# cesar-rocha/niwqg

Measured on NVIDIA B200. Metric: fp64 grid-point-steps/sec (coupled NIW-QG), higher is better.
Workload: dtype f64

## Files before the change

### niwqg_b200/csrc/common.cuh

```cuda
#pragma once
#include <cuda_runtime.h>
#include "fft_core.cuh"

#define NIWQG_PW_THREADS 256
#define NIWQG_PW_BLOCKS (148 * 4)

__host__ __device__ __forceinline__ int sidx(int i, int N) { return i < (N >> 1) ? i : i - N; }

struct Grid {
    int N;
    double dk;
    int ncl;
    int h;
    int rank;
    int sym;
};
__host__ __device__ __forceinline__ int grid_kx(const Grid& g, int lc) {
    if (!g.sym) return lc;
    if (lc < g.h) return g.rank * g.h + lc;
    if (g.rank == 0 && lc == g.h) return g.N >> 1;
    return g.N - (g.rank * g.h + lc - g.h);
}
__host__ __device__ __forceinline__ int grid_partner(const Grid& g, int lc) {
    if (!g.sym) return (g.N - lc) & (g.N - 1);
    if (g.rank == 0 && (lc == 0 || lc == g.h)) return lc;
    return lc < g.h ? lc + g.h : lc - g.h;
}
__host__ __device__ __forceinline__ void grid_owner(int N, int h, int kx, int& rank, int& lc) {
    const int H = N >> 1;
    if (kx < H) { rank = kx / h; lc = kx % h; }
    else if (kx == H) { rank = 0; lc = h; }
    else { const int m = N - kx; rank = m / h; lc = h + m % h; }
}

template <int K>
__device__ __forceinline__ void block_reduce_store(double (&s)[K], double* __restrict__ partials) {
    __shared__ double sh[NIWQG_PW_THREADS / 32][K];
    const int lane = threadIdx.x & 31, warp = threadIdx.x >> 5;
#pragma unroll
    for (int k = 0; k < K; ++k) {
        double x = s[k];
#pragma unroll
        for (int off = 16; off > 0; off >>= 1) x += __shfl_down_sync(0xffffffffu, x, off);
        if (lane == 0) sh[warp][k] = x;
    }
    __syncthreads();
    if (threadIdx.x < K) {
        double x = 0.0;
#pragma unroll
        for (int w = 0; w < NIWQG_PW_THREADS / 32; ++w) x += sh[w][threadIdx.x];
        partials[((size_t)blockIdx.y * gridDim.x + blockIdx.x) * K + threadIdx.x] = x;
    }
}

template <int K>
__device__ __forceinline__ void block_reduce_max_store(double (&s)[K], double* __restrict__ partials) {
    __shared__ double shm[NIWQG_PW_THREADS / 32][K];
    const int lane = threadIdx.x & 31, warp = threadIdx.x >> 5;
#pragma unroll
    for (int k = 0; k < K; ++k) {
        double x = s[k];
#pragma unroll
        for (int off = 16; off > 0; off >>= 1) x = fmax(x, __shfl_down_sync(0xffffffffu, x, off));
        if (lane == 0) shm[warp][k] = x;
    }
    __syncthreads();
// ... 8 lines not shown
```

### niwqg_b200/csrc/fft2d.cuh

```cuda
#pragma once
#include <cooperative_groups.h>
#include <cuda.h>
#include "common.cuh"

namespace cg = cooperative_groups;

enum {
    PRO_NONE = 0,
    PRO_REAL_IN,
    PRO_IK,
    PRO_IL,
    PRO_NEG_WV2,
    PRO_WV4,
    PRO_UV,
    PRO_IK_CONJ,
    PRO_IL_CONJ,
};
enum { EPI_NONE = 0, EPI_REAL_OUT };

struct FftArgs {
    const void* in;
    void* out;
    const cd* tw;
    const cd* twc;
    int pro, epi;
    int conj_in, conj_out;
    double scale, scale_im;
    double dk;
    int pf_groups;
    Grid g;
    int nlines;
    int pitch;
    int xmap_in, xmap_out;
    int xchunk;
    int deint_in, deint_out;
    int push;
    int nyl_shift;
    int panel;
    cd* peer[8];
    size_t mstride;
    int tma_in;
    int one_cta_per_sm;
    int variant;
    const cd *in2, *in3;
    double ld_scale;
};
enum {
    LD_NONE = 0,
    LD_WAVEPV,
    LD_UQVQ,
};

__device__ __forceinline__ size_t panel_offset(const FftArgs& a, int yl, int lc) {
    int cs = 0;
    while ((1 << cs) < a.panel) ++cs;
    const int rp = ((yl & (a.panel - 1)) << (a.nyl_shift - cs)) | (yl >> cs);
    return ((((size_t)(lc >> 2)) << a.nyl_shift) + rp) * 4 + (lc & 3);
}

template <int N, bool COL, bool NAT>
__device__ __forceinline__ size_t fft_index(const FftArgs& a, int xmap, int line, int n) {
    if (NAT) return COL ? (size_t)n * N + line : (size_t)line * N + n;
    if (COL) return (size_t)n * a.pitch + line;
    if (!xmap) return (size_t)line * N + n;
    int r, lc;
    grid_owner(N, a.g.h, n, r, lc);
    if (a.panel) return (size_t)r * a.xchunk + panel_offset(a, line, lc);
    return (size_t)r * a.xchunk + (size_t)line * a.g.ncl + lc;
}
template <bool COL>
__device__ __forceinline__ void fft_kykx(const FftArgs& a, int line, int n, int& ky, int& kx) {
    if (COL) { ky = n; kx = a.g.sym ? grid_kx(a.g, line) : line; } else { ky = line; kx = n; }
}

template <int N, int PRO>
__device__ __forceinline__ cd fft_prologue_one(const FftArgs& a, int row, int col, cd x) {
    const double k = a.dk * (double)sidx(col, N), l = a.dk * (double)sidx(row, N);
    if (PRO == PRO_IK) return make_double2(-k * x.y, k * x.x);
    if (PRO == PRO_IL) return make_double2(-l * x.y, l * x.x);
    if (PRO == PRO_IL_CONJ) return make_double2(l * x.y, -l * x.x);
    if (PRO == PRO_IK_CONJ) return make_double2(k * x.y, -k * x.x);
    if (PRO == PRO_NEG_WV2) { const double w = -(k * k + l * l); return make_double2(w * x.x, w * x.y); }
    if (PRO == PRO_WV4) { double w = k * k + l * l; w = w * w; return make_double2(w * x.x, w * x.y); }
// ... 172 lines not shown
        const cd* __restrict__ p2 = a.in3 + i0;
#pragma unroll
        for (int b = 0; b < fftc::E; b += 4) {
            cd x0[4], x1[4], x2[4];
#pragma unroll
            for (int i = 0; i < 4; ++i) {
                x0[i] = __ldg(p0 + (b + i) * TL::TPF); x1[i] = __ldg(p1 + (b + i) * TL::TPF); x2[i] = __ldg(p2 + (b + i) * TL::TPF);
            }
#pragma unroll
            for (int i = 0; i < 4; ++i) {
                const double im = x1[i].x * x2[i].y - x1[i].y * x2[i].x;
                v[b + i] = make_double2(x0[i].x * x0[i].x + x0[i].y * x0[i].y, a.ld_scale * (-2.0 * im));
            }
        }
        for (int t = tid; t < TL::TWLEN; t += TL::T) smtw[t] = a.tw[t];
        tma_done = true;
    }
    if constexpr (LD == LD_UQVQ) {
        static_assert(!COL && NAT && C == 1, "loader passes are one-tile row passes");
        const size_t i0 = mbase + (size_t)group * W * N + (size_t)w * M + j;
        const cd* __restrict__ p0 = (const cd*)a.in + i0;
        const cd* __restrict__ p1 = a.in2 + i0;
#pragma unroll
        for (int b = 0; b < fftc::E; b += 8) {
            cd x0[8], x1[8];
#pragma unroll
            for (int i = 0; i < 8; ++i) { x0[i] = __ldg(p0 + (b + i) * TL::TPF); x1[i] = __ldg(p1 + (b + i) * TL::TPF); }
#pragma unroll
            for (int i = 0; i < 8; ++i) v[b + i] = make_double2(x0[i].x * x1[i].x, x0[i].y * x1[i].x);
        }
        for (int t = tid; t < TL::TWLEN; t += TL::T) smtw[t] = a.tw[t];
        tma_done = true;
    }
    if constexpr (LD == LD_NONE && COL && NAT && C == 1 && M >= 256) {
        if (a.tma_in & 1) {
            const unsigned bar = smem_u32(smtw + TL::TWLEN);
            if (tid == 0) {
                mbar_init(bar, 1);
                asm volatile("fence.proxy.async.shared::cta;" ::: "memory");
            }
            __syncthreads();
            if (tid == 0) {
                mbar_expect_tx(bar, (unsigned)(W * M * sizeof(cd)));
#pragma unroll
                for (int b4 = 0; b4 < M / 256; ++b4)
                    tma_load_2d(smem_u32(smem + (size_t)b4 * 256 * W), &tmap, group * W * 2, (int)blockIdx.y * N + b4 * 256, bar);
            }
            for (int t = tid; t < TL::TWLEN; t += TL::T) smtw[t] = a.tw[t];
            mbar_wait(bar, 0);
#pragma unroll
            for (int e = 0; e < fftc::E; ++e) v[e] = smem[(size_t)(j + e * TL::TPF) * W + w];
            __syncthreads();
            tma_done = true;
        }
    }
    if constexpr (LD == LD_NONE && !COL && NAT && C == 1 && M * W == 4096) {
        if ((a.tma_in & 2) && a.pro != PRO_REAL_IN) {
            const unsigned bar = smem_u32(smtw + TL::TWLEN);
            if (tid == 0) {
                mbar_init(bar, 1);
                asm volatile("fence.proxy.async.shared::cta;" ::: "memory");
            }
            __syncthreads();
            if (tid == 0) {
                mbar_expect_tx(bar, (unsigned)(W * M * sizeof(cd)));
                bulk_load(smem_u32(smem), (const cd*)a.in + mbase + (size_t)group * W * N, (unsigned)(W * M * sizeof(cd)), bar);
// ... 426 lines not shown
```

### niwqg_b200/csrc/fft_split.cuh

```cuda
#pragma once
#include "fft2d.cuh"

struct SplitPArgs {
    const cd* in;
    cd* out[3];
    int pro[3];
    int nout;
    int conj_in;
    double scale;
    double dk;
    const cd* twc;
};

template <int N, int PRO>
__device__ __forceinline__ cd split_prologue(double dk, int row, int col, cd x) {
    FftArgs a{};
    a.dk = dk;
    return fft_prologue_one<N, PRO>(a, row, col, x);
}

template <int N, bool DIT>
__global__ void __launch_bounds__(256, 2) k_split_p(SplitPArgs a) {
    constexpr int R = 16, M = N / R, Nh = N / 2;
    const int lane = threadIdx.x & 31, warp = threadIdx.x >> 5;
// ... 56 lines not shown
            fftc::apply_twiddles<R, 1>(u, wy);
        }
        cd* out = a.out[o];
#pragma unroll
        for (int q = 0; q < R; ++q) {
            cd x = u[q];
            if (DIT) { x.x *= a.scale; x.y *= a.scale; }
            out[(size_t)(DIT ? m + M * q : q * M + m) * N + col] = x;
        }
    }
}

template <int M, int W, int R, bool DIT>
__global__ void __launch_bounds__(W * M / 16, 2) k_fft_colsub2(FftArgs a) {
    using TL = Tile<M, W, R, true>;
    constexpr int N = TL::N;
    extern __shared__ __align__(128) unsigned char smem_raw[];
    cd* smem = reinterpret_cast<cd*>(smem_raw);
    cd* smtw = smem + (size_t)W * TL::LINE;
    const int tid = threadIdx.x, w = tid % W, j = tid / W;
    const int q = (int)(blockIdx.x % R), group = (int)(blockIdx.x / R);
    const int line = group * W + w;
    const cd* in = (const cd*)a.in;
    cd v[fftc::E];
#pragma unroll
    for (int e = 0; e < fftc::E; ++e) {
        const int jj = j + e * TL::TPF;
        v[e] = in[(size_t)(DIT ? R * jj + q : q * M + jj) * N + line];
    }
    for (int t = tid; t < TL::TWLEN; t += TL::T) smtw[t] = a.tw[t];
    fft_stages<M, W, R, true, true, true, 1>(v, j, w, q, smem, smtw, a, line, 0);
}

template <int N>
static cudaError_t split_set_attrs() {
    constexpr int M = N / 16, W = 4096 / M;
    using TL = Tile<M, W, 16, true>;
    static bool attr_set[64] = {};
    int dev = 0;
    cudaGetDevice(&dev);
    if (dev < 64 && !attr_set[dev]) {
        cudaError_t e = cudaFuncSetAttribute(k_fft_colsub2<M, W, 16, false>, cudaFuncAttributeMaxDynamicSharedMemorySize, (int)TL::SMEM);
        if (e != cudaSuccess) return e;
        e = cudaFuncSetAttribute(k_fft_colsub2<M, W, 16, true>, cudaFuncAttributeMaxDynamicSharedMemorySize, (int)TL::SMEM);
        if (e != cudaSuccess) return e;
        attr_set[dev] = true;
    }
    return cudaSuccess;
}

template <int N, bool DIT>
static cudaError_t launch_split_colsub(const FftArgs& a, cudaStream_t st) {
    constexpr int M = N / 16, W = 4096 / M;
    using TL = Tile<M, W, 16, true>;
    cudaError_t e = split_set_attrs<N>();
    if (e != cudaSuccess) return e;
    FftArgs b = a;
    b.deint_out = DIT ? 1 : 0;
    k_fft_colsub2<M, W, 16, DIT><<<dim3((N / W) * 16, 1), TL::T, TL::SMEM, st>>>(b);
    return cudaGetLastError();
}

template <int N, int LD>
static cudaError_t launch_split_rows_loader(const FftArgs& a, cudaStream_t st) {
    constexpr int Nh = N / 2, W = 4096 / Nh;
    using TL = Tile<Nh, W, 1, false>;
    static bool attr_set[64] = {};
    int dev = 0;
    cudaGetDevice(&dev);
    if (dev >= 64 || !attr_set[dev]) {
        cudaError_t e = cudaFuncSetAttribute(k_fft_pass<Nh, W, 1, false, true, LD>, cudaFuncAttributeMaxDynamicSharedMemorySize, (int)TL::SMEM);
        if (e != cudaSuccess) return e;
        if (dev < 64) attr_set[dev] = true;
    }
    CUtensorMap tmap;
    memset(&tmap, 0, sizeof tmap);
    FftArgs b = a;
    b.tma_in = 0; b.pf_groups = 0;
    k_fft_pass<Nh, W, 1, false, true, LD><<<dim3(a.nlines / W, 1, 1), TL::T, TL::SMEM, st>>>(b, tmap);
    return cudaGetLastError();
}

template <int N, bool DIT>
static cudaError_t launch_split_p(const SplitPArgs& a, cudaStream_t st) {
    k_split_p<N, DIT><<<dim3(N / 2 / 128, N / 16, 1), 256, 0, st>>>(a);
    return cudaGetLastError();
}
```

### niwqg_b200/csrc/kernels_family.cuh

```cuda
#pragma once
#include "common.cuh"

enum {
    MF_WAVE_PV   = 1 << 0,
    MF_QL_ADV    = 1 << 1,
    MF_YBJ       = 1 << 2,
    MF_FIX00     = 1 << 3,
    MF_HAS_LAP2  = 1 << 4,
    MF_NO_WRITE  = 1 << 5,
    MF_SKIP_P1   = 1 << 6,
    MF_SKIP_P2   = 1 << 7,
    MF_SPEC_BUDGET = 1 << 8,
    MF_P1_BY_LOADER = 1 << 9,
};


__device__ __forceinline__ cd cexp_d(cd z) {
    double s, c;
    sincos(z.y, &s, &c);
    const double e = exp(z.x);
    return make_double2(e * c, e * s);
}
__device__ __forceinline__ cd cdiv_d(cd a, cd b) {
    if (fabs(b.x) >= fabs(b.y)) {
        const double r = b.y / b.x, d = b.x + b.y * r;
        return make_double2((a.x + a.y * r) / d, (a.y - a.x * r) / d);
    } else {
        const double r = b.x / b.y, d = b.x * r + b.y;
        return make_double2((a.x * r + a.y) / d, (a.y * r - a.x) / d);
    }
}

__device__ void etdrk4_point(cd ch, double dt, cd& E, cd& E2, cd& Q, cd& f0, cd& fab, cd& fc) {
    E = cexp_d(ch);
    E2 = cexp_d(make_double2(0.5 * ch.x, 0.5 * ch.y));
    cd sQ = make_double2(0, 0), s0 = sQ, sab = sQ, sc = sQ;
    for (int jj = 1; jj <= 32; ++jj) {
        double sr, cr;
        sincospi(2.0 * (double)jj / 32.0, &sr, &cr);
        const cd LR = make_double2(ch.x + cr, ch.y + sr);
        const cd LR2 = cmul(LR, LR), LR3 = cmul(LR2, LR);
        const cd eh = cexp_d(make_double2(0.5 * LR.x, 0.5 * LR.y));
        const cd e1 = cexp_d(LR);
        sQ = cadd(sQ, cdiv_d(make_double2(eh.x - 1.0, eh.y), LR));
        cd t = cmul(e1, make_double2(4.0 - 3.0 * LR.x + LR2.x, -3.0 * LR.y + LR2.y));
        s0 = cadd(s0, cdiv_d(make_double2(-4.0 - LR.x + t.x, -LR.y + t.y), LR3));
// ... 139 lines not shown
        if (a.qwh) a.qwh[i1] = make_double2(qwb.x * fl1, qwb.y * fl1);
        if (!self) {
            a.ph[i2] = make_double2(ph1.x, -ph1.y);
            a.qs[i2] = make_double2(Hq.x + qw.y, -Hq.y + qw.x);
            if (a.qwh) a.qwh[i2] = make_double2(qwb.x * fl2, -qwb.y * fl2);
        }
    }
    if (a.partials) block_reduce_store<SI_COUNT>(s, a.partials);
}

__global__ void k_spec_uvq(Grid g, const cd* __restrict__ qh, cd* __restrict__ uvq) {
    const int N = g.N, H = N >> 1, NC = g.ncl;
    const size_t npts = (size_t)N * NC, mb = (size_t)blockIdx.y * npts;
    const size_t total = (size_t)(H + 1) * NC;
    for (size_t t = (size_t)blockIdx.x * blockDim.x + threadIdx.x; t < total; t += (size_t)gridDim.x * blockDim.x) {
        const int ky = (int)(t / NC), lc = (int)(t % NC);
        const int kyp = (N - ky) & (N - 1), lcp = grid_partner(g, lc);
        if (kyp == ky && lcp < lc) continue;
        const int kx = grid_kx(g, lc), kxp = grid_kx(g, lcp);
        const size_t i1 = mb + (size_t)ky * NC + lc, i2 = mb + (size_t)kyp * NC + lcp;
        const double k1 = g.dk * (double)sidx(kx, N), l1 = g.dk * (double)sidx(ky, N);
        const double k2 = g.dk * (double)sidx(kxp, N), l2 = g.dk * (double)sidx(kyp, N);
        const double wv2 = __dadd_rn(__dmul_rn(k1, k1), __dmul_rn(l1, l1));
        const double wv2i = (wv2 != 0.0) ? 1.0 / wv2 : 0.0;
        const cd q1 = qh[i1], q2 = qh[i2];
        const cd G1 = make_double2(-wv2i * q1.x, -wv2i * q1.y), G2 = make_double2(-wv2i * q2.x, -wv2i * q2.y);
        cd o1, o2;
        pack_uv_general(k1, l1, k2, l2, G1, G2, o1, o2);
        uvq[i1] = o1;
        if (i1 != i2) uvq[i2] = o2;
    }
}

enum {
    SD_G1 = 0,
    SD_G2,
    SD_X1,
    SD_X2,
    SD_PHI_R, SD_PHI_I,
    SD_QPC_R, SD_QPC_I,
    SD_PHI2,
    SD_GRAD2,
    SD_LAP2,
    SD_J_R, SD_J_I,
    SD_Q2,
    SD_QP2,
    SD_QP3,
    SD_COUNT
};

struct PhysArgs {
    size_t npts;
    int flags;
    double nu4w, nuw, muw;
    const cd *uv, *qs, *phi, *phix, *phiy, *lapphi, *lap2phi, *uvq;
    cd *P1, *P2;
    double* partials;
};

__global__ void __launch_bounds__(NIWQG_PW_THREADS) k_phys_rhs(PhysArgs a) {
    const size_t mb = (size_t)blockIdx.y * a.npts;
    double s[SD_COUNT];
#pragma unroll
    for (int k = 0; k < SD_COUNT; ++k) s[k] = 0.0;
    const bool ybj = (a.flags & MF_YBJ) != 0, wr = !(a.flags & MF_NO_WRITE);
    const bool nosums = ybj || (a.flags & MF_SKIP_P1);
    for (size_t i = (size_t)blockIdx.x * blockDim.x + threadIdx.x; i < a.npts; i += (size_t)gridDim.x * blockDim.x) {
        const cd uv = a.uv[mb + i], qs = a.qs[mb + i];
        const cd phi = a.phi[mb + i], px = a.phix[mb + i], py = a.phiy[mb + i];
        const double u = uv.x, v = uv.y, q = qs.x, qpsi = qs.x - qs.y;
        const cd J = make_double2(u * px.x + v * py.x, u * px.y + v * py.y);
        cd Jadv = J;
        if (a.flags & MF_QL_ADV) {
            const cd w = a.uvq[mb + i];
            Jadv = make_double2(w.x * px.x + w.y * py.x, w.x * px.y + w.y * py.y);
        }
        if (wr) {
            if (!ybj && !(a.flags & (MF_SKIP_P1 | MF_P1_BY_LOADER))) a.P1[mb + i] = make_double2(u * q, v * q);
            if (!(a.flags & MF_SKIP_P2))
                a.P2[mb + i] = make_double2(-Jadv.x + 0.5 * phi.y * qpsi, -Jadv.y - 0.5 * phi.x * qpsi);
        }
        if (nosums) continue;
        s[SD_PHI_R] += phi.x; s[SD_PHI_I] += phi.y;
        s[SD_QPC_R] += qpsi * phi.x; s[SD_QPC_I] += -qpsi * phi.y;
        s[SD_PHI2] += phi.x * phi.x + phi.y * phi.y;
        s[SD_GRAD2] += px.x * px.x + px.y * px.y + py.x * py.x + py.y * py.y;
        s[SD_J_R] += Jadv.x; s[SD_J_I] += Jadv.y;
        s[SD_Q2] += q * q;
        s[SD_QP2] += qpsi * qpsi;
        s[SD_QP3] += qpsi * qpsi * qpsi;
        if (a.flags & MF_SPEC_BUDGET) continue;
        const cd lp = a.lapphi[mb + i];
        cd diss = make_double2(a.nuw * lp.x - a.muw * phi.x, a.nuw * lp.y - a.muw * phi.y);
        if (a.flags & MF_HAS_LAP2) {
            const cd l2 = a.lap2phi[mb + i];
            diss.x += -a.nu4w * l2.x; diss.y += -a.nu4w * l2.y;
        }
        s[SD_G1] += qpsi * (phi.x * lp.y - phi.y * lp.x);
        s[SD_G2] += lp.x * J.x + lp.y * J.y;
        s[SD_X1] += -(diss.y * J.x - diss.x * J.y);
        s[SD_X2] += 0.5 * (diss.x * phi.x + diss.y * phi.y) * qpsi;
        s[SD_LAP2] += lp.x * lp.x + lp.y * lp.y;
    }
    if (!nosums) block_reduce_store<SD_COUNT>(s, a.partials);
}

__global__ void __launch_bounds__(256) k_finalize(const double* __restrict__ partials, int nblk, int K, double* __restrict__ out, int is_max) {
    __shared__ double sh[16][17];
    const int m = blockIdx.x, k = threadIdx.x & 15, part = threadIdx.x >> 4;
    const double* p = partials + (size_t)m * nblk * K;
    double x = is_max ? -1.0e300 : 0.0;
// ... 282 lines not shown
```

### niwqg_b200/csrc/niwqg_b200.cu

```cuda
#include <cstdio>
#include <cstdlib>
#include <cstring>
#include <cmath>
#include <string>
#include <vector>
#include <dlfcn.h>
#include <nccl.h>
#include "../../include/niwqg_b200.h"
#include "fft2d.cuh"
#include "fft_split.cuh"
#include "kernels_family.cuh"
#include "kernels_fused.cuh"
#include "kernels_qg.cuh"
#include "kernels_ic.cuh"

static std::string g_create_error;

#define CK(call)                                                                                   \
    do {                                                                                           \
        cudaError_t e__ = (call);                                                                  \
        if (e__ != cudaSuccess) {                                                                  \
            char buf__[512];                                                                       \
            snprintf(buf__, sizeof buf__, "%s:%d: %s: %s", __FILE__, __LINE__, #call, cudaGetErrorString(e__)); \
            h->err = buf__;                                                                        \
            return -2;                                                                             \
        }                                                                                          \
    } while (0)

struct niwqg_handle {
    niwqg_params p;
    int N = 0, B = 1, model = 0, flags = 0;
    bool qg = false;
// ... 17 lines not shown
    cd *ph = nullptr, *qwh = nullptr;
    cd *phi = nullptr, *phix = nullptr, *phiy = nullptr, *lapphi = nullptr, *lap2phi = nullptr;
    cd *uv = nullptr, *qs = nullptr, *uvq = nullptr;
    cd *W = nullptr, *P1 = nullptr, *P2 = nullptr;
    double* rscratch = nullptr;
    double *part = nullptr, *sumsD = nullptr, *sumsE = nullptr, *sumsX = nullptr, *sumsI = nullptr, *scal = nullptr,
           *stagev = nullptr;
    bool q_set = false, phi_set = false;
    int deintC = 1, deintM = 0;
    int rank = 0, nranks = 1, nyl = 0, ncl = 0;
    Grid g{};
    double Mg = 0;
    cd *X = nullptr, *Y = nullptr;
    static constexpr int NLANE = 2;
    cd* Yp[NLANE][2] = {};
    cd* peerY[NLANE][2][8] = {};
    bool p2p = false;
    int ybuf[NLANE] = {0, 0};
    double* bar[NLANE] = {nullptr, nullptr};
    cudaStream_t lane_stream[NLANE] = {nullptr, nullptr};
    ncclComm_t lane_comm[NLANE] = {nullptr, nullptr};
    cudaEvent_t ev_fork = nullptr, ev_join = nullptr;
    struct StepGraph { cudaGraphExec_t exec = nullptr; int cq = 0, cp = 0, cc = 0; long long launches = 0; };
    StepGraph graphs[8];
    bool use_graphs = false;
    int direct_steps = 0;
    int exchange = 0;
    cd* Xl[NLANE] = {nullptr, nullptr};
    ncclComm_t comm = nullptr;
    bool col3 = false;
    cd* S3[2] = {nullptr, nullptr};
    cd* tw_c3 = nullptr;
    int split = 0;
    cd* T[3] = {nullptr, nullptr, nullptr};
    cd *tw_half = nullptr, *tw_m = nullptr;
    cudaStream_t copy_stream = nullptr, copy_out = nullptr;
    cudaEvent_t ev_up_done = nullptr, ev_up_free = nullptr, ev_dn_ready = nullptr, ev_dn_done[2] = {nullptr, nullptr};
    bool up_free_rec = false, dn_done_rec[2] = {false, false};
    void* stage_in = nullptr;
    void* pre_buf[2] = {nullptr, nullptr};
    cudaEvent_t pre_done[2] = {nullptr, nullptr}, pre_free[2] = {nullptr, nullptr};
    bool pre_staged[2] = {false, false}, pre_free_rec[2] = {false, false};
    void* stage_out[2] = {nullptr, nullptr};
    double* pin = nullptr;
    int slab_panel = 0;
    int flag_barrier = 1;
    unsigned bar_epoch[NLANE] = {0, 0};
    bool prof = false;
    struct ProfRec { int kind; cudaEvent_t a, b; };
    std::vector<ProfRec> prof_recs;
    std::vector<cudaEvent_t> prof_pool;
    size_t prof_used = 0;
};

enum { PK_FFT_ROW = 0, PK_FFT_COL, PK_PHYS, PK_SPEC, PK_SMALL, PK_COMM, PK_FFT_P, PK_FFT_ROWLD, PK_FFT_ROWLD2, PK_COUNT };

static cudaEvent_t prof_event(niwqg_handle* h) {
    if (h->prof_used == h->prof_pool.size()) {
        cudaEvent_t e;
        cudaEventCreate(&e);
        h->prof_pool.push_back(e);
    }
    return h->prof_pool[h->prof_used++];
}
struct ProfScope {
    niwqg_handle* h; int kind; cudaEvent_t a;
// ... 101 lines not shown
    const int r = threadIdx.x;
    if (r >= nranks) return;
    unsigned v;
    do {
        asm volatile("ld.acquire.sys.global.u32 %0, [%1];" : "=r"(v) : "l"(flags + r) : "memory");
        if (v < epoch) __nanosleep(200);
    } while (v < epoch);
}

static constexpr int WAVE_CTAS = 296;

static void fft_common_args(niwqg_handle* h, FftArgs& a) {
    a.twc = h->twc;
    a.dk = h->dk;
    a.pf_groups = WAVE_CTAS;
    a.variant = 6;
    a.one_cta_per_sm = 0;
    a.g = h->g;
    a.xmap_in = a.xmap_out = 0;
    a.deint_in = a.deint_out = 0;
    a.tma_in = 1;
    a.xchunk = h->nyl * h->ncl;
    a.mstride = h->npts;
    a.pitch = h->ncl;
}

static int split_rows(niwqg_handle* h, const void* in, void* out, int pro, int epi, double sc, bool conj_out) {
    FftArgs a{};
    fft_common_args(h, a);
    const int Nh = h->N / 2;
    a.in = in; a.out = out; a.pro = pro; a.epi = epi; a.tw = h->tw_half;
    a.nlines = 2 * h->N; a.pitch = Nh; a.mstride = (size_t)Nh * Nh; a.g = Grid{Nh, h->dk, Nh, Nh / 2, 0, 0};
    a.conj_in = 0; a.conj_out = conj_out ? 1 : 0; a.scale = sc; a.scale_im = conj_out ? -sc : sc;
    a.tma_in = 2;
    a.pf_groups = 0;
    { PROF(PK_FFT_ROW); CK(launch_pass<false>(Nh, a, 1, h->stream)); }
    h->launches++;
    return 0;
}
static int split_rows_loader(niwqg_handle* h, int ld, cd* out) {
    FftArgs a{};
    fft_common_args(h, a);
    const int Nh = h->N / 2;
    if (ld == LD_WAVEPV) { a.in = h->phi; a.in2 = h->phix; a.in3 = h->phiy; a.ld_scale = h->jscale; }
    else { a.in = h->uv; a.in2 = h->qs; a.in3 = nullptr; a.ld_scale = 1.0; }
    a.out = out; a.pro = PRO_NONE; a.epi = EPI_NONE; a.tw = h->tw_half;
    a.nlines = 2 * h->N; a.pitch = Nh; a.mstride = (size_t)Nh * Nh; a.g = Grid{Nh, h->dk, Nh, Nh / 2, 0, 0};
    a.conj_in = 0; a.conj_out = 0; a.scale = 1.0; a.scale_im = 1.0;
    cudaError_t e = cudaErrorInvalidValue;
    {
        PROF(ld == LD_WAVEPV ? PK_FFT_ROWLD : PK_FFT_ROWLD2);
#define NIWQG_LD_CASE(NN) case NN: e = (ld == LD_WAVEPV) ? launch_split_rows_loader<NN, LD_WAVEPV>(a, h->stream) \
                                                          : launch_split_rows_loader<NN, LD_UQVQ>(a, h->stream); break;
        switch (h->N) {
            NIWQG_LD_CASE(2048)
            NIWQG_LD_CASE(4096)
            NIWQG_LD_CASE(8192)
        }
#undef NIWQG_LD_CASE
    }
    CK(e);
    h->launches++;
    return 0;
}
static int split_colsub(niwqg_handle* h, const cd* in, cd* out, bool dit) {
    FftArgs a{};
    fft_common_args(h, a);
    a.in = in; a.out = out; a.pro = PRO_NONE; a.epi = EPI_NONE; a.tw = h->tw_m; a.scale = 1.0; a.scale_im = 1.0;
    cudaError_t e = cudaErrorInvalidValue;
    {
        PROF(PK_FFT_COL);
        switch (h->N) {
            case 2048: e = dit ? launch_split_colsub<2048, true>(a, h->stream) : launch_split_colsub<2048, false>(a, h->stream); break;
            case 4096: e = dit ? launch_split_colsub<4096, true>(a, h->stream) : launch_split_colsub<4096, false>(a, h->stream); break;
            case 8192: e = dit ? launch_split_colsub<8192, true>(a, h->stream) : launch_split_colsub<8192, false>(a, h->stream); break;
        }
    }
    CK(e);
    h->launches++;
    return 0;
}
static int split_p(niwqg_handle* h, const cd* in, cd* const* out, const int* pro, int nout, bool dit, bool conj_in) {
    SplitPArgs p{};
    p.in = in; p.nout = nout; p.conj_in = conj_in ? 1 : 0; p.scale = 1.0; p.dk = h->dk; p.twc = h->twc;
    for (int o = 0; o < nout; ++o) { p.out[o] = out[o]; p.pro[o] = pro[o]; }
    cudaError_t e = cudaErrorInvalidValue;
// ... 184 lines not shown
        return 0;
    }
    SlabFlags f{};
    for (int r = 0; r < h->nranks; ++r) f.peer[r] = (unsigned*)(h->peerY[lane][0][r] + h->npts);
    const unsigned epoch = ++h->bar_epoch[lane];
    k_slab_signal<<<1, 32, 0, st>>>(f, h->nranks, h->rank, epoch);
    k_slab_wait<<<1, 32, 0, st>>>((const unsigned*)(h->Yp[lane][0] + h->npts), h->nranks, epoch);
    CK(cudaGetLastError());
    return 0;
}

#define FFT(...)                          \
    do {                                  \
        int r__ = fft2(h, __VA_ARGS__);   \
        if (r__) return r__;              \
    } while (0)

struct FftJob { const void* in; cd* out; bool inverse; int pro; };
static int fft2_group(niwqg_handle* h, const FftJob* jobs, int n) {
    const bool par = (h->p2p || h->nranks == 1) && !h->prof && n > 1 && !h->split;
    if (!par) {
        for (int i = 0; i < n; ++i) FFT(jobs[i].in, jobs[i].out, jobs[i].inverse, jobs[i].pro, h->B);
        return 0;
    }
    CK(cudaEventRecord(h->ev_fork, h->lane_stream[0]));
    CK(cudaStreamWaitEvent(h->lane_stream[1], h->ev_fork, 0));
    for (int i = 0; i < n; ++i) FFT(jobs[i].in, jobs[i].out, jobs[i].inverse, jobs[i].pro, h->B, EPI_NONE, nullptr, i & 1);
    CK(cudaEventRecord(h->ev_join, h->lane_stream[1]));
    CK(cudaStreamWaitEvent(h->lane_stream[0], h->ev_join, 0));
    return 0;
}

static int finalize(niwqg_handle* h, int K, double* out, int is_max = 0, int nblk = NIWQG_PW_BLOCKS) {
    PROF(PK_SMALL);
    k_finalize<<<h->B, 256, 0, h->stream>>>(h->part, nblk, K, out, is_max);
    CK(cudaGetLastError());
    h->launches += 1;
    if (h->nranks > 1)
        NK(g_nccl.AllReduce(out, out, (size_t)h->B * K, ncclDouble, is_max ? ncclMax : ncclSum, h->comm, h->stream));
    return 0;
}
#define FIN(...)                              \
    do {                                      \
        int r__ = finalize(h, __VA_ARGS__);   \
        if (r__) return r__;                  \
    } while (0)

__global__ void k_budget(BudgetArgs a) {
    const int m = blockIdx.x;
    if (threadIdx.x != 0) return;
    const double* sd = a.sumsD + (size_t)m * SD_COUNT;
    const double* se = a.sumsE + (size_t)m * SE_COUNT;
    const double* si = a.sumsI + (size_t)m * SI_COUNT;
    double* sc = a.scal + (size_t)m * NIWQG_S_COUNT;
    const double M = a.M, M2 = M * M;
    double g1, g2, x1, x2, lap2m;
    if (a.spec_budget) {
        g1 = 0.5 * a.hslash * (se[SE_T1R] / M2) / a.f;
        g2 = 0.0;
        x1 = ((-a.nu4w * se[SE_T2I] - a.nuw * se[SE_T1I] - a.muw * se[SE_T0I]) / M2) / a.f;
        x2 = 0.0;
        lap2m = se[SE_LAP2] / M2;
    } else {
        g1 = 0.5 * 0.5 * a.hslash * (sd[SD_G1] / M) / a.f;
        g2 = 0.5 * a.hslash * (sd[SD_G2] / M) / a.f;
        x1 = (sd[SD_X1] / M) / a.f; x2 = (sd[SD_X2] / M) / a.f;
// ... 122 lines not shown
        const FftJob jobs[2] = {FftJob{h->ph, h->uv, true, PRO_UV}, FftJob{h->qs, h->qs, true, PRO_NONE}};
        int r = fft2_group(h, jobs, 2);
        if (r) return r;
    }
    return 0;
}

static PhysArgs phys_args(niwqg_handle* h, int extra_flags) {
    PhysArgs pa{};
    pa.npts = h->npts; pa.flags = h->flags | extra_flags;
    pa.nu4w = h->p.nu4w; pa.nuw = h->p.nuw; pa.muw = h->p.muw;
    pa.uv = h->uv; pa.qs = h->qs; pa.phi = h->phi; pa.phix = h->phix; pa.phiy = h->phiy;
    pa.lapphi = h->lapphi; pa.lap2phi = h->lap2phi; pa.uvq = h->uvq;
    pa.P1 = h->P1; pa.P2 = h->P2; pa.partials = h->part;
    return pa;
}

static int ql_wave_velocity(niwqg_handle* h) {
    { PROF(PK_SPEC); k_spec_uvq<<<pw_grid(h), NIWQG_PW_THREADS, 0, h->stream>>>(h->g, h->qh[h->cq], h->uvq); }
    CK(cudaGetLastError());
    h->launches++;
    FFT(h->uvq, h->uvq, true, PRO_NONE, h->B);
    return 0;
}

template <int N>
static int step_family_fused_n(niwqg_handle* h) {
    const int oq = h->cq, op = h->cp, nq = 1 - oq, np = 1 - op;
    const bool wave = (h->flags & MF_WAVE_PV) != 0;
    const double sc = 1.0 / ((double)N * (double)N);
    const int grid = WAVE_CTAS;
    int r;
    for (int st = 1; st <= 4; ++st) {
        PhysArgs pa = phys_args(h, MF_P1_BY_LOADER);
        { PROF(PK_PHYS); k_phys_rhs<<<pw_grid(h), NIWQG_PW_THREADS, 0, h->stream>>>(pa); }
        CK(cudaGetLastError());
        h->launches++;
        FIN(SD_COUNT, h->sumsD);
        if ((r = split_rows_loader(h, LD_UQVQ, h->P1))) return r;
        if ((r = split_colsub(h, h->P1, h->T[0], true))) return r;
        if ((r = split_rows(h, h->P2, h->P2, PRO_NONE, EPI_NONE, 1.0, false))) return r;
        if ((r = split_colsub(h, h->P2, h->T[1], true))) return r;
        FStageArgs fa{};
        StageArgs& sa = fa.s;
        sa.g = h->g; sa.stage = st; sa.flags = h->flags; sa.do_q = 1; sa.do_phi = 1; sa.sums_here = 1;
        sa.P1 = h->P1; sa.P2 = h->P2;
        sa.y0q = h->qh[oq]; sa.y0p = h->phih[op]; sa.yq = h->qh[nq]; sa.yp = h->phih[np];
        sa.y1q = h->y1q; sa.y1p = h->y1p; sa.F0q = h->F0q; sa.F0p = h->F0p; sa.Fabq = h->Fabq; sa.Fabp = h->Fabp;
        if (st == 1) { sa.yq = h->y1q; sa.yp = h->y1p; }
        sa.ph = h->ph; sa.tq = h->tq; sa.tp = h->tp; sa.filtr = h->filtr; sa.sumsD = h->sumsD; sa.partials = h->part;
        fa.twc = h->twc; fa.dk = h->dk;
        sa.hsym = (h->p.use_filter || !h->p.dealias) ? 1 : 0;
        fa.T = h->T[0];
        { PROF(PK_SPEC); CK((launch_fstage<N>(fa, false, grid, h->stream))); }
        fa.T = h->T[1];
        fa.out[0] = h->T[1]; fa.out[1] = h->T[2]; fa.out[2] = h->T[0];
        fa.nout = wave ? 3 : 1;
        { PROF(PK_SPEC); CK((launch_fstage<N>(fa, true, grid, h->stream))); }
        h->launches += 2;
        if (st == 1) { h->cq = nq; h->cp = np; }
        FIN(SE_COUNT, h->sumsE, 0, grid);
        { PROF(PK_SMALL); k_budget<<<h->B, 32, 0, h->stream>>>(budget_args(h, st)); }
        CK(cudaGetLastError());
        h->launches++;
        if ((r = split_colsub(h, h->T[1], h->phi, false))) return r;
        if ((r = split_rows(h, h->phi, h->phi, PRO_NONE, EPI_NONE, sc, true))) return r;
        if (wave) {
            if ((r = split_colsub(h, h->T[2], h->phix, false))) return r;
            if ((r = split_rows(h, h->phix, h->phix, PRO_NONE, EPI_NONE, sc, true))) return r;
            if ((r = split_colsub(h, h->T[0], h->phiy, false))) return r;
            if ((r = split_rows(h, h->phiy, h->phiy, PRO_NONE, EPI_NONE, sc, true))) return r;
            if ((r = split_rows_loader(h, LD_WAVEPV, h->W))) return r;
            if ((r = split_colsub(h, h->W, h->T[0], true))) return r;
        }
// ... 306 lines not shown
    for (void* p : h->allocs) cudaFree(p);
    for (cudaEvent_t e : h->prof_pool) cudaEventDestroy(e);
    if (h->copy_stream) { cudaStreamSynchronize(h->copy_stream); cudaStreamDestroy(h->copy_stream); }
    if (h->copy_out) { cudaStreamSynchronize(h->copy_out); cudaStreamDestroy(h->copy_out); }
    for (cudaEvent_t e : {h->ev_up_done, h->ev_up_free, h->ev_dn_ready, h->ev_dn_done[0], h->ev_dn_done[1]}) if (e) cudaEventDestroy(e);
    for (int w = 0; w < 2; ++w) {
        if (h->pre_buf[w]) cudaFree(h->pre_buf[w]);
        if (h->pre_done[w]) cudaEventDestroy(h->pre_done[w]);
        if (h->pre_free[w]) cudaEventDestroy(h->pre_free[w]);
    }
    if (h->pin) cudaFreeHost(h->pin);
    if (h->ev0) cudaEventDestroy(h->ev0);
    if (h->ev1) cudaEventDestroy(h->ev1);
    if (h->stream) cudaStreamDestroy(h->stream);
    delete h;
    return 0;
}

static int create_impl(niwqg_handle* h) {
    const niwqg_params& p = h->p;
    const int N = p.nx;
    CK(cudaSetDevice(p.device));
    CK(cudaStreamCreateWithFlags(&h->stream, cudaStreamNonBlocking));
    CK(cudaEventCreate(&h->ev0));
    CK(cudaEventCreate(&h->ev1));
    CK(cudaStreamCreateWithFlags(&h->copy_stream, cudaStreamNonBlocking));
    CK(cudaStreamCreateWithFlags(&h->copy_out, cudaStreamNonBlocking));
    CK(cudaEventCreateWithFlags(&h->ev_up_done, cudaEventDisableTiming));
    CK(cudaEventCreateWithFlags(&h->ev_up_free, cudaEventDisableTiming));
    CK(cudaEventCreateWithFlags(&h->ev_dn_ready, cudaEventDisableTiming));
    CK(cudaEventCreateWithFlags(&h->ev_dn_done[0], cudaEventDisableTiming));
    CK(cudaEventCreateWithFlags(&h->ev_dn_done[1], cudaEventDisableTiming));
    h->N = N; h->B = p.batch; h->model = p.model; h->qg = (p.model == NIWQG_MODEL_QG);
    CK(cudaMallocHost((void**)&h->pin, ((size_t)p.batch * (NIWQG_S_COUNT + 64) + 64) * sizeof(double)));
    h->nranks = p.nranks > 1 ? p.nranks : 1;
    h->rank = h->nranks > 1 ? p.rank : 0;
    h->nyl = N / h->nranks; h->ncl = N / h->nranks;
    h->nk = h->qg ? N / 2 + 1 : h->ncl;
    h->npts = (size_t)h->nyl * N; h->nspec = (size_t)N * h->nk;
    h->Mg = (double)N * (double)N;
    if (h->nranks == 1 && h->B == 1 && !h->qg && N >= 2048) {
        const char* e = getenv("NIWQG_SPLIT");
        h->split = e ? (atoi(e) != 0) : (N == 8192);
        if (h->split) { h->deintM = N / 2; h->deintC = 2; }
    }
    h->col3 = h->nranks == 1 && N == 8192 && h->B == 1 && !h->split;
    h->g = Grid{N, 2.0 * M_PI / p.L, h->ncl, h->ncl / 2, h->rank, h->nranks > 1 ? 1 : 0};
    if (h->nranks > 1) {
        int r = nccl_load(h->err);
        if (r) return r;
        ncclUniqueId id;
        memcpy(&id, p.nccl_id, sizeof id);
        NK(g_nccl.CommInitRank(&h->comm, h->nranks, id, h->rank));
    }
    h->dk = 2.0 * M_PI / p.L; h->dx = p.L / N;
    {
        const double kmid = h->dk * N / 8.0;
        h->jscale = exp2(rint(log2(1.0 / (kmid * kmid))));
    }
    if (!h->qg) {
        const double kappa = p.m * p.f / p.N;
        h->kappa2 = kappa * kappa;
        h->hslash = p.f / h->kappa2;
    }
    switch (p.model) {
        case NIWQG_MODEL_COUPLED: h->flags = MF_WAVE_PV | MF_FIX00 | MF_SPEC_BUDGET; break;
// ... 76 lines not shown
        DA(h->S3[0], fsz); DA(h->S3[1], fsz);
        std::vector<cd> tw3;
        build_twiddles(512, tw3);
        DA(h->tw_c3, tw3.size() * cb);
        CK(cudaMemcpyAsync(h->tw_c3, tw3.data(), tw3.size() * cb, cudaMemcpyHostToDevice, h->stream));
        CK(cudaStreamSynchronize(h->stream));
    }
    CK(cudaStreamCreateWithFlags(&h->lane_stream[1], cudaStreamNonBlocking));
    CK(cudaEventCreateWithFlags(&h->ev_fork, cudaEventDisableTiming));
    CK(cudaEventCreateWithFlags(&h->ev_join, cudaEventDisableTiming));
    if (h->nranks > 1) {
        DA(h->X, fsz); DA(h->Y, fsz);
        h->slab_panel = (N >= NIWQG_COL_M && h->nyl >= N / NIWQG_COL_M && h->ncl % 4 == 0) ? N / NIWQG_COL_M : 0;
        for (int l = 0; l < niwqg_handle::NLANE; ++l) { DA(h->Yp[l][0], fsz + 4096); DA(h->Yp[l][1], fsz); DA(h->bar[l], 64); DA(h->Xl[l], fsz); }
        if (const char* e = getenv("NIWQG_SLAB_BARRIER")) h->flag_barrier = strcmp(e, "nccl") != 0;
        if (const char* e = getenv("NIWQG_SLAB_EXCHANGE")) h->exchange = (strcmp(e, "ce") == 0) ? 1 : 0;
        NK(g_nccl.CommSplit(h->comm, 0, h->rank, &h->lane_comm[1], nullptr));
    }
    if (p.model != NIWQG_MODEL_YBJ) { DA(h->qh[1], ssz); DA(h->y1q, ssz); DA(h->F0q, ssz); DA(h->Fabq, ssz); }
    if (!h->qg) {
        DA(h->phih[0], ssz); DA(h->phih[1], ssz); DA(h->y1p, ssz); DA(h->F0p, ssz); DA(h->Fabp, ssz);
        DA(h->phi, fsz); DA(h->phix, fsz); DA(h->phiy, fsz); DA(h->lapphi, fsz);
        if (h->flags & MF_HAS_LAP2) DA(h->lap2phi, fsz);
        if (h->flags & MF_WAVE_PV) DA(h->qwh, ssz);
        if (h->flags & MF_QL_ADV) DA(h->uvq, fsz);
    } else if (p.passive_scalar) {
        DA(h->chh[0], ssz); DA(h->chh[1], ssz); DA(h->y1c, ssz); DA(h->F0c, ssz); DA(h->Fabc, ssz);
    }
    if (B * h->npts * sizeof(cd) >= STAGED_BYTES) {
        DA(h->stage_in, B * h->npts * sizeof(cd));
        DA(h->stage_out[0], h->npts * sizeof(double));
        DA(h->stage_out[1], h->npts * sizeof(cd));
    }
    DA(h->part, B * NIWQG_PW_BLOCKS * 16 * sizeof(double));
    DA(h->sumsD, B * 16 * sizeof(double)); DA(h->sumsE, B * 16 * sizeof(double)); DA(h->sumsX, B * 16 * sizeof(double));
    DA(h->sumsI, B * 16 * sizeof(double));
    DA(h->scal, B * NIWQG_S_COUNT * sizeof(double)); DA(h->stagev, B * 24 * sizeof(double));
    CK(cudaStreamSynchronize(h->stream));
    return 0;
}

int niwqg_create(const niwqg_params* p, niwqg_handle** out) {
    if (!p || !out) { g_create_error = "null argument"; return -1; }
    *out = nullptr;
    if (p->struct_size != sizeof(niwqg_params)) {
        g_create_error = "niwqg_params.struct_size does not match this library (binding built against another header)";
        return -1;
    }
    const int N = p->nx;
    if (N < 32 || N > 8192 || (N & (N - 1))) { g_create_error = "nx must be a power of two in [32, 8192]"; return -1; }
    if (p->batch < 1) { g_create_error = "batch must be >= 1"; return -1; }
    if (p->model < NIWQG_MODEL_QG || p->model > NIWQG_MODEL_QL) { g_create_error = "unknown model"; return -1; }
    if (p->nranks > 1) {
        const int P = p->nranks;
        if ((P & (P - 1)) || N / P < 16 || p->rank < 0 || p->rank >= P) { g_create_error = "slab: nranks must be a power of two with nx/nranks >= 16, 0 <= rank < nranks"; return -1; }
        if (p->model == NIWQG_MODEL_QG) { g_create_error = "slab: QGModel (half spectrum) is single-GPU only"; return -1; }
        if (p->batch != 1) { g_create_error = "slab: batch must be 1 (ensembles shard whole members per GPU instead)"; return -1; }
    }
    int ndev = 0;
    if (cudaGetDeviceCount(&ndev) != cudaSuccess || ndev == 0) {
        g_create_error = "no CUDA device: niwqg_b200 has no CPU fallback";
        return -3;
    }
    niwqg_handle* h = new niwqg_handle();
    h->p = *p;
    int r = create_impl(h);
    if (r) { g_create_error = h->err; niwqg_destroy(h); return r; }
// ... 734 lines not shown
```

Baseline: 1.285 billion.

## Fuse physical-space RHS and diagnostic sums into the P2 row-FFT loader

Removes the separate k_phys_rhs pointwise kernel in the split path. The nonlinear P2 term and the diagnostic partial sums are now computed inside a new LD_P2 loader of the row FFT pass, which also drops one separate row FFT pass over P2. This avoids writing P2 to global memory and reading it back. Because the partial sums now come from many more CTAs, a two-level finalize reduction and a larger partials buffer are added. That reduction is restricted to one member and one rank, and the loader keeps more values live in registers.

```diff
diff --git a/niwqg_b200/csrc/common.cuh b/niwqg_b200/csrc/common.cuh
--- a/niwqg_b200/csrc/common.cuh
+++ b/niwqg_b200/csrc/common.cuh
@@ -32,6 +32,23 @@
     else if (kx == H) { rank = 0; lc = h; }
     else { const int m = N - kx; rank = m / h; lc = h + m % h; }
 }
+
+enum {
+    SD_G1 = 0,
+    SD_G2,
+    SD_X1,
+    SD_X2,
+    SD_PHI_R, SD_PHI_I,
+    SD_QPC_R, SD_QPC_I,
+    SD_PHI2,
+    SD_GRAD2,
+    SD_LAP2,
+    SD_J_R, SD_J_I,
+    SD_Q2,
+    SD_QP2,
+    SD_QP3,
+    SD_COUNT
+};
 
 template <int K>
 __device__ __forceinline__ void block_reduce_store(double (&s)[K], double* __restrict__ partials) {
diff --git a/niwqg_b200/csrc/fft2d.cuh b/niwqg_b200/csrc/fft2d.cuh
--- a/niwqg_b200/csrc/fft2d.cuh
+++ b/niwqg_b200/csrc/fft2d.cuh
@@ -44,11 +44,14 @@
     int variant;
     const cd *in2, *in3;
     double ld_scale;
+    const cd *in4, *in5;
+    double* partials;
 };
 enum {
     LD_NONE = 0,
     LD_WAVEPV,
     LD_UQVQ,
+    LD_P2,
 };
 
 __device__ __forceinline__ size_t panel_offset(const FftArgs& a, int yl, int lc) {
@@ -287,6 +290,45 @@
         for (int t = tid; t < TL::TWLEN; t += TL::T) smtw[t] = a.tw[t];
         tma_done = true;
     }
+    if constexpr (LD == LD_P2) {
+        static_assert(!COL && NAT && C == 1, "loader passes are one-tile row passes");
+        static_assert(TL::T == NIWQG_PW_THREADS, "block_reduce_store reduces over NIWQG_PW_THREADS threads");
+        const size_t i0 = mbase + (size_t)line * N + j;
+        const cd* __restrict__ puv = (const cd*)a.in + i0;
+        const cd* __restrict__ pqs = a.in2 + i0;
+        const cd* __restrict__ pph = a.in3 + i0;
+        const cd* __restrict__ ppx = a.in4 + i0;
+        const cd* __restrict__ ppy = a.in5 + i0;
+        double s[SD_COUNT];
+#pragma unroll
+        for (int k = 0; k < SD_COUNT; ++k) s[k] = 0.0;
+#pragma unroll
+        for (int b = 0; b < fftc::E; b += 2) {
+            cd uv[2], qs[2], phi[2], px[2], py[2];
+#pragma unroll
+            for (int i = 0; i < 2; ++i) {
+                const int o = (b + i) * TL::TPF;
+                uv[i] = __ldg(puv + o); qs[i] = __ldg(pqs + o); phi[i] = __ldg(pph + o); px[i] = __ldg(ppx + o); py[i] = __ldg(ppy + o);
+            }
+#pragma unroll
+            for (int i = 0; i < 2; ++i) {
+                const double u = uv[i].x, vv = uv[i].y, q = qs[i].x, qpsi = qs[i].x - qs[i].y;
+                const cd J = make_double2(u * px[i].x + vv * py[i].x, u * px[i].y + vv * py[i].y);
+                v[b + i] = make_double2(-J.x + 0.5 * phi[i].y * qpsi, -J.y - 0.5 * phi[i].x * qpsi);
+                s[SD_PHI_R] += phi[i].x; s[SD_PHI_I] += phi[i].y;
+                s[SD_QPC_R] += qpsi * phi[i].x; s[SD_QPC_I] += -qpsi * phi[i].y;
+                s[SD_PHI2] += phi[i].x * phi[i].x + phi[i].y * phi[i].y;
+                s[SD_GRAD2] += px[i].x * px[i].x + px[i].y * px[i].y + py[i].x * py[i].x + py[i].y * py[i].y;
+                s[SD_J_R] += J.x; s[SD_J_I] += J.y;
+                s[SD_Q2] += q * q;
+                s[SD_QP2] += qpsi * qpsi;
+                s[SD_QP3] += qpsi * qpsi * qpsi;
+            }
+        }
+        block_reduce_store<SD_COUNT>(s, a.partials);
+        for (int t = tid; t < TL::TWLEN; t += TL::T) smtw[t] = a.tw[t];
+        tma_done = true;
+    }
     if constexpr (LD == LD_NONE && COL && NAT && C == 1 && M >= 256) {
         if (a.tma_in & 1) {
             const unsigned bar = smem_u32(smtw + TL::TWLEN);
diff --git a/niwqg_b200/csrc/fft_split.cuh b/niwqg_b200/csrc/fft_split.cuh
--- a/niwqg_b200/csrc/fft_split.cuh
+++ b/niwqg_b200/csrc/fft_split.cuh
@@ -141,6 +141,8 @@
     return cudaGetLastError();
 }
 
+static inline int split_row_ctas(int N) { return (int)((size_t)N * N / 4096); }
+
 template <int N, int LD>
 static cudaError_t launch_split_rows_loader(const FftArgs& a, cudaStream_t st) {
     constexpr int Nh = N / 2, W = 4096 / Nh;
diff --git a/niwqg_b200/csrc/kernels_family.cuh b/niwqg_b200/csrc/kernels_family.cuh
--- a/niwqg_b200/csrc/kernels_family.cuh
+++ b/niwqg_b200/csrc/kernels_family.cuh
@@ -11,7 +11,6 @@
     MF_SKIP_P1   = 1 << 6,
     MF_SKIP_P2   = 1 << 7,
     MF_SPEC_BUDGET = 1 << 8,
-    MF_P1_BY_LOADER = 1 << 9,
 };
 
 
@@ -217,22 +216,6 @@
     }
 }
 
-enum {
-    SD_G1 = 0,
-    SD_G2,
-    SD_X1,
-    SD_X2,
-    SD_PHI_R, SD_PHI_I,
-    SD_QPC_R, SD_QPC_I,
-    SD_PHI2,
-    SD_GRAD2,
-    SD_LAP2,
-    SD_J_R, SD_J_I,
-    SD_Q2,
-    SD_QP2,
-    SD_QP3,
-    SD_COUNT
-};
 
 struct PhysArgs {
     size_t npts;
@@ -261,7 +244,7 @@
             Jadv = make_double2(w.x * px.x + w.y * py.x, w.x * px.y + w.y * py.y);
         }
         if (wr) {
-            if (!ybj && !(a.flags & (MF_SKIP_P1 | MF_P1_BY_LOADER))) a.P1[mb + i] = make_double2(u * q, v * q);
+            if (!ybj && !(a.flags & MF_SKIP_P1)) a.P1[mb + i] = make_double2(u * q, v * q);
             if (!(a.flags & MF_SKIP_P2))
                 a.P2[mb + i] = make_double2(-Jadv.x + 0.5 * phi.y * qpsi, -Jadv.y - 0.5 * phi.x * qpsi);
         }
diff --git a/niwqg_b200/csrc/niwqg_b200.cu b/niwqg_b200/csrc/niwqg_b200.cu
--- a/niwqg_b200/csrc/niwqg_b200.cu
+++ b/niwqg_b200/csrc/niwqg_b200.cu
@@ -1,3 +1,4 @@
+#include <algorithm>
 #include <cstdio>
 #include <cstdlib>
 #include <cstring>
@@ -259,15 +260,17 @@
     fft_common_args(h, a);
     const int Nh = h->N / 2;
     if (ld == LD_WAVEPV) { a.in = h->phi; a.in2 = h->phix; a.in3 = h->phiy; a.ld_scale = h->jscale; }
-    else { a.in = h->uv; a.in2 = h->qs; a.in3 = nullptr; a.ld_scale = 1.0; }
+    else if (ld == LD_UQVQ) { a.in = h->uv; a.in2 = h->qs; a.ld_scale = 1.0; }
+    else { a.in = h->uv; a.in2 = h->qs; a.in3 = h->phi; a.in4 = h->phix; a.in5 = h->phiy; a.partials = h->part; a.ld_scale = 1.0; }
     a.out = out; a.pro = PRO_NONE; a.epi = EPI_NONE; a.tw = h->tw_half;
     a.nlines = 2 * h->N; a.pitch = Nh; a.mstride = (size_t)Nh * Nh; a.g = Grid{Nh, h->dk, Nh, Nh / 2, 0, 0};
     a.conj_in = 0; a.conj_out = 0; a.scale = 1.0; a.scale_im = 1.0;
     cudaError_t e = cudaErrorInvalidValue;
     {
-        PROF(ld == LD_WAVEPV ? PK_FFT_ROWLD : PK_FFT_ROWLD2);
+        PROF(ld == LD_UQVQ ? PK_FFT_ROWLD2 : PK_FFT_ROWLD);
 #define NIWQG_LD_CASE(NN) case NN: e = (ld == LD_WAVEPV) ? launch_split_rows_loader<NN, LD_WAVEPV>(a, h->stream) \
-                                                          : launch_split_rows_loader<NN, LD_UQVQ>(a, h->stream); break;
+                                     : (ld == LD_UQVQ) ? launch_split_rows_loader<NN, LD_UQVQ>(a, h->stream)     \
+                                                       : launch_split_rows_loader<NN, LD_P2>(a, h->stream); break;
         switch (h->N) {
             NIWQG_LD_CASE(2048)
             NIWQG_LD_CASE(4096)
@@ -518,6 +521,20 @@
 }
 
 static int finalize(niwqg_handle* h, int K, double* out, int is_max = 0, int nblk = NIWQG_PW_BLOCKS) {
+    if (nblk > NIWQG_PW_BLOCKS) {
+        if (h->B != 1 || h->nranks != 1 || nblk % 128 != 0) {
+            h->err = "finalize: two-level reduction needs one member, one rank and a multiple of 128 partial sets";
+            return -1;
+        }
+        const int groups = nblk / 128;
+        double* grp = h->part + (size_t)nblk * K;
+        { PROF(PK_SMALL); k_finalize<<<groups, 256, 0, h->stream>>>(h->part, 128, K, grp, is_max); }
+        CK(cudaGetLastError());
+        { PROF(PK_SMALL); k_finalize<<<1, 256, 0, h->stream>>>(grp, groups, K, out, is_max); }
+        CK(cudaGetLastError());
+        h->launches += 2;
+        return 0;
+    }
     PROF(PK_SMALL);
     k_finalize<<<h->B, 256, 0, h->stream>>>(h->part, nblk, K, out, is_max);
     CK(cudaGetLastError());
@@ -706,14 +723,10 @@
     const int grid = WAVE_CTAS;
     int r;
     for (int st = 1; st <= 4; ++st) {
-        PhysArgs pa = phys_args(h, MF_P1_BY_LOADER);
-        { PROF(PK_PHYS); k_phys_rhs<<<pw_grid(h), NIWQG_PW_THREADS, 0, h->stream>>>(pa); }
-        CK(cudaGetLastError());
-        h->launches++;
-        FIN(SD_COUNT, h->sumsD);
+        if ((r = split_rows_loader(h, LD_P2, h->P2))) return r;
+        FIN(SD_COUNT, h->sumsD, 0, split_row_ctas(N));
         if ((r = split_rows_loader(h, LD_UQVQ, h->P1))) return r;
         if ((r = split_colsub(h, h->P1, h->T[0], true))) return r;
-        if ((r = split_rows(h, h->P2, h->P2, PRO_NONE, EPI_NONE, 1.0, false))) return r;
         if ((r = split_colsub(h, h->P2, h->T[1], true))) return r;
         FStageArgs fa{};
         StageArgs& sa = fa.s;
@@ -1228,7 +1241,7 @@
         DA(h->stage_out[0], h->npts * sizeof(double));
         DA(h->stage_out[1], h->npts * sizeof(cd));
     }
-    DA(h->part, B * NIWQG_PW_BLOCKS * 16 * sizeof(double));
+    DA(h->part, B * std::max(NIWQG_PW_BLOCKS, h->split ? split_row_ctas(N) / 128 * 129 : 0) * 16 * sizeof(double));
     DA(h->sumsD, B * 16 * sizeof(double)); DA(h->sumsE, B * 16 * sizeof(double)); DA(h->sumsX, B * 16 * sizeof(double));
     DA(h->sumsI, B * 16 * sizeof(double));
     DA(h->scal, B * NIWQG_S_COUNT * sizeof(double)); DA(h->stagev, B * 24 * sizeof(double));
```

Result: faster. 1.328 billion (median of 6 runs) (+3.4%).

## Add persistent TMA ring-buffered row FFT kernel for split path

Applied to the files above, without the earlier changes.

Adds a persistent kernel that launches one CTA per SM, with two 256-thread groups each taking alternate tiles. A three-slot shared-memory ring is filled by bulk async loads tracked with mbarriers, so the load of the next tile overlaps the FFT stages of the current one. Split row FFTs without real input now use this kernel instead of the generic pass. The cost is more complex synchronisation (named barriers and empty/full mbarriers) and a prologue handling that may differ from the old path. Occupancy also drops to one large CTA per SM.

```diff
diff --git a/niwqg_b200/csrc/fft_split.cuh b/niwqg_b200/csrc/fft_split.cuh
--- a/niwqg_b200/csrc/fft_split.cuh
+++ b/niwqg_b200/csrc/fft_split.cuh
@@ -112,6 +112,123 @@
     fft_stages<M, W, R, true, true, true, 1>(v, j, w, q, smem, smtw, a, line, 0);
 }
 
+constexpr int PIPE_SLOTS = 3;
+
+struct PipeSched {
+    HD static int tile(int cta, int grid, int k) { return cta + k * grid; }
+    HD static int group(int k) { return k & 1; }
+    HD static int slot(int k) { return k % PIPE_SLOTS; }
+    HD static int tiles_of(int cta, int grid, int ntiles) { return cta < ntiles ? (ntiles - 1 - cta) / grid + 1 : 0; }
+};
+
+template <int M, int W> struct PipeGeom {
+    using TL = Tile<M, W, 1, false>;
+    static constexpr int SLOT = W * TL::LINE;
+    static constexpr int TWOFF = PIPE_SLOTS * SLOT;
+    static constexpr size_t SMEM = ((size_t)TWOFF + TL::TWLEN) * sizeof(cd) + 2 * PIPE_SLOTS * sizeof(unsigned long long);
+    static constexpr unsigned BYTES = (unsigned)(W * M * sizeof(cd));
+    static_assert(W * M == 4096 && TL::T == 256, "one tile = 256 threads x 16 points");
+    static_assert(SMEM <= 227 * 1024, "ring does not fit in shared memory");
+};
+
+__device__ __forceinline__ void group_sync(int g) { asm volatile("bar.sync %0, 256;" ::"r"(1 + g) : "memory"); }
+__device__ __forceinline__ void mbar_arrive(unsigned bar) { asm volatile("mbarrier.arrive.shared::cta.b64 _, [%0];" ::"r"(bar) : "memory"); }
+
+template <int M, int W>
+__device__ __forceinline__ void pipe_issue(const FftArgs& a, int t, cd* dst, unsigned full) {
+    mbar_expect_tx(full, PipeGeom<M, W>::BYTES);
+    bulk_load(smem_u32(dst), (const cd*)a.in + (size_t)t * W * M, PipeGeom<M, W>::BYTES, full);
+}
+
+template <int M, int W, int NS, class Release, class Emit>
+__device__ __forceinline__ void pipe_stages(cd (&v)[fftc::E], int j, int w, int g, cd* slot, const cd* tw, Release&& release,
+                                            Emit&& emit) {
+    using TL = Tile<M, W, 1, false>;
+    constexpr int R = fftc::StageRadix<M, NS>::R;
+    constexpr int S = fftc::E / R;
+    fftc::stage_compute<M, NS>(v, j, tw);
+    if constexpr (NS * R == M) {
+#pragma unroll
+        for (int u = 0; u < S; ++u)
+#pragma unroll
+            for (int p = 0; p < R; ++p) emit(fftc::stage_out_index<M, NS>(j, u, p), v[u + p * S]);
+    } else {
+        constexpr int NS2 = NS * R;
+#pragma unroll
+        for (int u = 0; u < S; ++u)
+#pragma unroll
+            for (int p = 0; p < R; ++p) slot[TL::slot(w, fftc::stage_out_index<M, NS>(j, u, p))] = v[u + p * S];
+        group_sync(g);
+#pragma unroll
+        for (int e = 0; e < fftc::E; ++e) v[e] = slot[TL::slot(w, j + e * TL::TPF)];
+        if constexpr (NS2 * fftc::StageRadix<M, NS2>::R == M) release();
+        else group_sync(g);
+        pipe_stages<M, W, NS2>(v, j, w, g, slot, tw, release, emit);
+    }
+}
+
+template <int M, int W>
+__global__ void __launch_bounds__(512, 1) k_fft_tile_pipe(FftArgs a, int ntiles) {
+    using PG = PipeGeom<M, W>;
+    using TL = typename PG::TL;
+    extern __shared__ __align__(128) unsigned char smem_raw[];
+    cd* smem = reinterpret_cast<cd*>(smem_raw);
+    cd* smtw = smem + PG::TWOFF;
+    const unsigned bar0 = smem_u32(smtw + TL::TWLEN);
+    const int tid = threadIdx.x, g = tid >> 8, gt = tid & 255;
+    const int cta = blockIdx.x, grid = gridDim.x;
+    const int nk = PipeSched::tiles_of(cta, grid, ntiles);
+    const int j = gt % TL::TPF, w = gt / TL::TPF;
+    if (tid == 0) {
+        for (int b = 0; b < 2 * PIPE_SLOTS; ++b) mbar_init(bar0 + 8 * b, 1);
+        asm volatile("fence.proxy.async.shared::cta;" ::: "memory");
+        for (int k = 0; k < PIPE_SLOTS && k < nk; ++k)
+            pipe_issue<M, W>(a, PipeSched::tile(cta, grid, k), smem + (size_t)PipeSched::slot(k) * PG::SLOT, bar0 + 8 * PipeSched::slot(k));
+    }
+    for (int t = tid; t < TL::TWLEN; t += 512) smtw[t] = a.tw[t];
+    __syncthreads();
+#pragma unroll 1
+    for (int k = g; k < nk; k += 2) {
+        const int s = PipeSched::slot(k), t = PipeSched::tile(cta, grid, k);
+        const int next = k + PIPE_SLOTS < nk ? PipeSched::tile(cta, grid, k + PIPE_SLOTS) : -1;
+        cd* slot = smem + (size_t)s * PG::SLOT;
+        if (k >= PIPE_SLOTS) mbar_wait(bar0 + 8 * (PIPE_SLOTS + s), (unsigned)((k - PIPE_SLOTS) / PIPE_SLOTS) & 1);
+        mbar_wait(bar0 + 8 * s, (unsigned)(k / PIPE_SLOTS) & 1);
+        cd v[fftc::E];
+#pragma unroll
+        for (int e = 0; e < fftc::E; ++e) v[e] = slot[(size_t)w * M + j + e * TL::TPF];
+        group_sync(g);
+        auto release = [&]() {
+            asm volatile("fence.proxy.async.shared::cta;" ::: "memory");
+            group_sync(g);
+            if (gt == 0 && next >= 0) {
+                pipe_issue<M, W>(a, next, slot, bar0 + 8 * s);
+                mbar_arrive(bar0 + 8 * (PIPE_SLOTS + s));
+            }
+        };
+        const int line = t * W + w;
+        pipe_stages<M, W, 1>(v, j, w, g, slot, smtw, release, [&](int n, cd x) { fft_store<M, false, true>(a, 0, line, n, x); });
+    }
+}
+
+template <int M>
+static cudaError_t launch_tile_pipe(const FftArgs& a, int nsm, cudaStream_t st) {
+    constexpr int W = 4096 / M;
+    using PG = PipeGeom<M, W>;
+    static bool attr_set[64] = {};
+    int dev = 0;
+    cudaGetDevice(&dev);
+    if (dev >= 64 || !attr_set[dev]) {
+        cudaError_t e = cudaFuncSetAttribute(k_fft_tile_pipe<M, W>, cudaFuncAttributeMaxDynamicSharedMemorySize, (int)PG::SMEM);
+        if (e != cudaSuccess) return e;
+        if (dev < 64) attr_set[dev] = true;
+    }
+    if (a.nlines % W) return cudaErrorInvalidValue;
+    const int ntiles = a.nlines / W, grid = ntiles < nsm ? ntiles : nsm;
+    k_fft_tile_pipe<M, W><<<grid, 512, PG::SMEM, st>>>(a, ntiles);
+    return cudaGetLastError();
+}
+
 template <int N>
 static cudaError_t split_set_attrs() {
     constexpr int M = N / 16, W = 4096 / M;
diff --git a/niwqg_b200/csrc/niwqg_b200.cu b/niwqg_b200/csrc/niwqg_b200.cu
--- a/niwqg_b200/csrc/niwqg_b200.cu
+++ b/niwqg_b200/csrc/niwqg_b200.cu
@@ -81,6 +81,7 @@
     cd* S3[2] = {nullptr, nullptr};
     cd* tw_c3 = nullptr;
     int split = 0;
+    int nsm = 0;
     cd* T[3] = {nullptr, nullptr, nullptr};
     cd *tw_half = nullptr, *tw_m = nullptr;
     cudaStream_t copy_stream = nullptr, copy_out = nullptr;
@@ -248,9 +249,21 @@
     a.in = in; a.out = out; a.pro = pro; a.epi = epi; a.tw = h->tw_half;
     a.nlines = 2 * h->N; a.pitch = Nh; a.mstride = (size_t)Nh * Nh; a.g = Grid{Nh, h->dk, Nh, Nh / 2, 0, 0};
     a.conj_in = 0; a.conj_out = conj_out ? 1 : 0; a.scale = sc; a.scale_im = conj_out ? -sc : sc;
-    a.tma_in = 2;
-    a.pf_groups = 0;
-    { PROF(PK_FFT_ROW); CK(launch_pass<false>(Nh, a, 1, h->stream)); }
+    cudaError_t e = cudaErrorInvalidValue;
+    {
+        PROF(PK_FFT_ROW);
+        if (pro == PRO_REAL_IN) {
+            a.pf_groups = 0;
+            e = launch_pass<false>(Nh, a, 1, h->stream);
+        } else {
+            switch (Nh) {
+                case 1024: e = launch_tile_pipe<1024>(a, h->nsm, h->stream); break;
+                case 2048: e = launch_tile_pipe<2048>(a, h->nsm, h->stream); break;
+                case 4096: e = launch_tile_pipe<4096>(a, h->nsm, h->stream); break;
+            }
+        }
+    }
+    CK(e);
     h->launches++;
     return 0;
 }
@@ -1086,6 +1099,7 @@
     CK(cudaEventCreateWithFlags(&h->ev_dn_done[0], cudaEventDisableTiming));
     CK(cudaEventCreateWithFlags(&h->ev_dn_done[1], cudaEventDisableTiming));
     h->N = N; h->B = p.batch; h->model = p.model; h->qg = (p.model == NIWQG_MODEL_QG);
+    CK(cudaDeviceGetAttribute(&h->nsm, cudaDevAttrMultiProcessorCount, p.device));
     CK(cudaMallocHost((void**)&h->pin, ((size_t)p.batch * (NIWQG_S_COUNT + 64) + 64) * sizeof(double)));
     h->nranks = p.nranks > 1 ? p.nranks : 1;
     h->rank = h->nranks > 1 ? p.rank : 0;
```

After: 1.273 billion before, 1.293 billion after (median of 6 runs). 1.02x the previous value.
